# philgzl/brever

Measured on AMD Instinct MI355X. Metric: utterances/sec (4 s @16 kHz) Conv-TasNet train, higher is better.
Workload: dtype bf16

## Files before the change

### brever_amd/csrc/common.cuh

```cuda
#pragma once
#include <hip/hip_runtime.h>
#include <stdint.h>

namespace brv {

typedef __attribute__((ext_vector_type(8))) __bf16 bf16x8;
typedef __attribute__((ext_vector_type(4))) __bf16 bf16x4;
typedef __attribute__((ext_vector_type(4))) short s16x4;
typedef __attribute__((ext_vector_type(16))) float f32x16;
typedef __attribute__((ext_vector_type(4))) float f32x4;

typedef uint16_t bf16_t;

constexpr int kWave = 64;
constexpr int kThreads = 256;

__device__ __forceinline__ float bf2f(bf16_t v) {
  return __uint_as_float(((uint32_t)v) << 16);
}
__device__ __forceinline__ bf16_t f2bf(float f) {
  __bf16 h = (__bf16)f;
  return __builtin_bit_cast(bf16_t, h);
}
typedef __bf16 bf16x2_t __attribute__((ext_vector_type(2)));
// ... 37 lines not shown
__device__ __forceinline__ uint4 buf_load16(__amdgpu_buffer_rsrc_t r, unsigned int off) {
  const u32x4 v = __builtin_amdgcn_raw_buffer_load_b128(r, (int)off, 0, 0);
  return make_uint4(v.x, v.y, v.z, v.w);
}
__device__ __forceinline__ void buf_store16(__amdgpu_buffer_rsrc_t r, unsigned int off, const uint4& q) {
  u32x4 v; v.x = q.x; v.y = q.y; v.z = q.z; v.w = q.w;
#ifndef BRV_STORE_AUX
#define BRV_STORE_AUX 0
#endif
  __builtin_amdgcn_raw_buffer_store_b128(v, r, (int)off, 0, BRV_STORE_AUX);
}
constexpr unsigned int kOob = 0xfffffff0u;

template <typename T>
__device__ __forceinline__ T wave_sum(T v) {
#pragma unroll
  for (int off = 32; off > 0; off >>= 1) v += __shfl_xor(v, off, 64);
  return v;
}

template <typename T>
__device__ __forceinline__ T block_sum(T v, T* scratch) {
  v = wave_sum(v);
  const int lane = threadIdx.x & 63, wid = threadIdx.x >> 6;
  __syncthreads();
  if (lane == 0) scratch[wid] = v;
  __syncthreads();
  T r = T(0);
  if (threadIdx.x == 0) r = scratch[0] + scratch[1] + scratch[2] + scratch[3];
  return r;
}

#ifndef BRV_NO_ATOMICS
#define BRV_NO_ATOMICS 0
#endif
__device__ __forceinline__ void atomic_add_f64(double* p, double v) {
  if (BRV_NO_ATOMICS & 1) return;
  __hip_atomic_fetch_add(p, v, __ATOMIC_RELAXED, __HIP_MEMORY_SCOPE_AGENT);
}
__device__ __forceinline__ void atomic_add_f32(float* p, float v) {
  if (BRV_NO_ATOMICS & 2) return;
  __hip_atomic_fetch_add(p, v, __ATOMIC_RELAXED, __HIP_MEMORY_SCOPE_AGENT);
}

constexpr int kStatStride = 32;
__host__ __device__ __forceinline__ constexpr long long stat_sum(long long b) { return b*kStatStride; }
__host__ __device__ __forceinline__ constexpr long long stat_sq(long long b) { return b*kStatStride + kStatStride/2; }
struct NormStat { float mean, rstd; };
__device__ __forceinline__ float rstd_f32(double v) {
  const float x = (float)v;
  const float r = __builtin_amdgcn_rsqf(x);
  return r*__builtin_fmaf(-0.5f*x*r, r, 1.5f);
}
__device__ __forceinline__ NormStat norm_stat(const double* stats, int b,
                                              double inv_n, float eps) {
  const double s = stats[stat_sum(b)], ss = stats[stat_sq(b)];
  const double mean = s*inv_n;
  double var = ss*inv_n - mean*mean;
  if (var < 0.0) var = 0.0;
  NormStat r;
  r.mean = (float)mean;
  r.rstd = rstd_f32(var + (double)eps);
  return r;
}

__device__ __forceinline__ void load8_masked(const float* p, int c0, int C, float (&v)[8]) {
  if (p != nullptr && c0 + 8 <= C) {
#pragma unroll
    for (int j = 0; j < 8; ++j) v[j] = p[c0 + j];
  } else if (p != nullptr) {
#pragma unroll
    for (int j = 0; j < 8; ++j) {
      const int c = c0 + j;
      const float x = p[c < C ? c : (C > 0 ? C - 1 : 0)];
      v[j] = c < C ? x : 0.f;
    }
  } else {
#pragma unroll
    for (int j = 0; j < 8; ++j) v[j] = 0.f;
  }
}

__host__ __device__ inline int round_up(int x, int m) { return (x + m - 1)/m*m; }
__host__ __device__ inline int ceil_div(int x, int m) { return (x + m - 1)/m; }

}

#define GRID_STRIDE(i, n) \
  for (long long i = (long long)blockIdx.x*256 + threadIdx.x; i < (n); i += (long long)gridDim.x*256)
```

### brever_amd/csrc/convtasnet.hip

```cpp
#include <hip/hip_runtime.h>
#include <stdio.h>
#include <stdlib.h>
#include <string.h>
#include <algorithm>
#include <string>
#include <vector>

#include "../../include/brever_hip.h"
#include "status.h"
#include "ctn_layout.h"
#include "gemm_rows.cuh"
#include "gemm_wgrad.cuh"
#include "gemm_ws.cuh"
#include "dwpw2_fused.cuh"
#include "gemm_wgrad_full.cuh"
#include "gemm_wgrad_full128.cuh"

constexpr int kWgSplit = 4;
#include "prep.cuh"
#include "tcn_kernels.cuh"
#include "bwd_fused.cuh"
#include "pw1_bwd.cuh"
#include "cln_kernels.cuh"

using namespace brv;

namespace {

inline long long align_up(long long x, long long a) { return (x + a - 1)/a*a; }

const brv_launch_opts kDefaultOpts = {sizeof(brv_launch_opts), 0u, 8, 0, nullptr};
thread_local const brv_launch_opts* t_opts = &kDefaultOpts;
struct OptsScope {
  const brv_launch_opts* prev;
  explicit OptsScope(const brv_launch_opts* o) : prev(t_opts) {
    t_opts = (o && o->size >= sizeof(brv_launch_opts)) ? o : &kDefaultOpts;
  }
  ~OptsScope() { t_opts = prev; }
  int check() const {
    const uint32_t unknown = t_opts->flags & ~BRV_OPT_KNOWN;
    if (!unknown) return 0;
    char bits[16]; snprintf(bits, sizeof(bits), "0x%x", unknown);
    return fail(-1, std::string("unknown option bits ") + bits + " in brv_launch_opts.flags");
  }
};
inline bool opt(uint32_t flag) { return (t_opts->flags & flag) != 0; }
inline bool fwd_fuse_requested() { return !opt(BRV_OPT_NO_FWD_FUSE) && !opt(BRV_OPT_NO_WS); }
inline bool bwd_fuse_requested() { return !opt(BRV_OPT_NO_BWD_FUSE); }
inline bool pw1_rc_requested() { return !opt(BRV_OPT_NO_PW1_RC) && !opt(BRV_OPT_NO_DZ1_FUSE); }
inline bool pw1_rc_wgrad() { return opt(BRV_OPT_PW1_RC_WGRAD) || opt(BRV_OPT_PW1_RC_TILES); }

struct ProfEntry { const char* label; hipEvent_t a, b; double flops, bytes; };
struct Prof { std::vector<ProfEntry> entries; bool by_dil; };
struct ProfScope {
  hipStream_t st; Prof* prof;
  ProfScope(const char* label, double flops, double bytes, hipStream_t s)
      : st(s), prof(static_cast<Prof*>(t_opts->prof)) {
    if (!prof) return;
    ProfEntry e; e.label = label; e.flops = flops; e.bytes = bytes;
    (void)hipEventCreate(&e.a); (void)hipEventCreate(&e.b);
    (void)hipEventRecord(e.a, st);
    prof->entries.push_back(e);
  }
  ~ProfScope() { if (prof) (void)hipEventRecord(prof->entries.back().b, st); }
};
inline bool prof_by_dil() { return t_opts->prof && static_cast<Prof*>(t_opts->prof)->by_dil; }

struct BlockOff : CtnBlockOff {
  long long p_c1_f, p_c1_b, p_rs_f, p_rs_b;
  long long p_c1_fp, p_rs_fp, p_rs_bp;
  long long p_rs_g, p_rs_gp, p_lazy;
};

struct Layout : CtnLayout<BlockOff> {
  int Np, Kfp, Bnp, Hp, Scp;
  long long p_enc, p_dec_f, p_dec_b, p_bott_f, p_bott_b, p_out_f, p_out_b, p_stamp, n_prepared;

  bool fusable() const {
    return !causal && P == 3 && H == 512 && Bn == 128 && Sc == 128 && nb <= 24 ;
  }
  bool fused_fwd() const { return fusable() && fwd_fuse_requested(); }
  bool pw1_rc() const { return !causal && Hp == RC_H && Bnp == RC_N && pw1_rc_requested(); }

  static int limits(const brv_ctn_config* c) {
    return c->kernel_size < 1 || c->kernel_size > 5 ? fail(-2, "kernel_size must be in [1, 5] in the HIP path") : 0;
  }
  int init(const brv_ctn_config* c) {
    if (int r = CtnLayout::init(c, limits)) return r;
    Np = round_up(N, 64); Kfp = round_up(K, 64); Bnp = round_up(Bn, 64);
    Hp = round_up(H, 64); Scp = round_up(Sc, 64);
    long long q = 0;
    auto ptake = [&](long long n) { long long r = q; q += align_up(n, 128); return r; };
    p_enc = ptake((long long)Np*Kfp);
    p_dec_f = ptake((long long)Kfp*Np);
    p_dec_b = ptake((long long)Np*Kfp);
    p_bott_f = ptake((long long)Bnp*Np);
    p_bott_b = ptake((long long)Np*Bnp);
    for (int i = 0; i < nb; ++i) {
      const int rs = (i < nb - 1 ? Bnp : 0) + Scp;
      blk[i].p_c1_f = ptake((long long)Hp*Bnp);
      blk[i].p_c1_b = ptake((long long)Bnp*Hp);
      blk[i].p_rs_f = ptake((long long)rs*Hp);
      blk[i].p_rs_b = ptake((long long)Hp*rs);
      blk[i].p_c1_fp = ptake((long long)Hp*Bnp);
      blk[i].p_rs_fp = ptake((long long)rs*Hp);
      blk[i].p_rs_bp = ptake((long long)Hp*rs);
      blk[i].p_rs_g = ptake((long long)(Bnp + Scp)*Hp);
      blk[i].p_rs_gp = ptake((long long)(Bnp + Scp)*Hp);
      blk[i].p_lazy = ptake(4LL*(Bnp + Scp));
    }
    p_out_f = ptake((long long)S*Np*Scp);
    p_out_b = ptake((long long)Scp*S*Np);
    p_stamp = ptake(128);
    n_prepared = q;
    return 0;
  }
};

struct Workspace {
  long long w, x, z1, z2, skip, m, y, stats, sums, dpre, dw1, gskip, gout, eA, eB,
      e0, dwt, vg, gcopy, total;
  long long gcopy_stride, eB_stride;
  long long wgpart;
  long long h1, h2, wn, ctab, ctab_stride, cfs, cbt, ident, fake_stats, scratch_stats;
  long long vg_stride, vg_bytes;
  long long x_stride, z_stride;
  long long u, u_stride;
  long long stamp;
  long long stats_bytes;
  void init(const Layout& l, long long B, long long T) {
    long long o = 0;
    auto take = [&](long long bytes) { long long r = o; o += align_up(bytes, 256); return r; };
    const long long BT = B*T;
    w = take(BT*l.Np*2);
    x_stride = align_up(BT*l.Bnp*2, 256);
    x = take(x_stride*l.nb);
    z_stride = align_up(BT*l.Hp*2, 256);
    z1 = take(z_stride*l.nb);
    z2 = take(z_stride*l.nb);
    skip = take(BT*l.Scp*4);
    m = take(BT*l.S*l.Np*2);
    y = take(BT*l.S*l.Np*2);
    stats_bytes = (long long)(1 + 2*l.nb)*B*kStatStride*8;
    stats = take(stats_bytes);
    sums = take(stats_bytes);
    dpre = take(BT*l.S*l.Np*2);
    dw1 = take(BT*l.S*l.Np*2);
    gout = take(BT*(l.Bnp + l.Scp)*2);
    gskip = gout + (long long)l.Bnp*2;
    eA = take(BT*l.Hp*2);
    eB_stride = align_up(BT*l.Hp*2, 256);
    eB = take(eB_stride*l.nb);
    gcopy_stride = align_up(BT*l.Bnp*2, 256);
    gcopy = take(gcopy_stride*l.nb);
    e0 = take(BT*l.Np*2);
    dwt = take(BT*l.Np*2);
    vg_stride = align_up(2LL*l.N + (long long)l.nb*l.H*(5 + l.P) + 1 + 2*l.nb + 2LL*l.Hp, 64);
    vg_bytes = vg_stride*kReplicas*4;
    vg = take(vg_bytes);
    wgpart = take((long long)2*kWgSplit*l.nb*W2_G*l.H*4);
    u_stride = align_up(BT*(l.Bnp + l.Scp)*2, 256);
    u = l.fusable() ? take(u_stride*l.nb) : 0;
// ... 978 lines not shown
    g.e.src = v.z2(i); g.e.ld_src = l.Hp; g.e.src_slope = params + b.prelu2;
    g.e.src_stats = v.stat(2 + 2*i); g.e.inv_n = 1.0/((double)T*l.H); g.e.eps = 1e-8f;
    g.e.gamma = params + b.n2_g;
    g.e.dgamma = v.vslot(i) + 2*l.H; g.e.dbeta = v.vslot(i) + 3*l.H;
    g.e.rep_stride = v.ws.vg_stride; g.e.n_rep = kReplicas;
    g.e.sums_out = v.sum(2 + 2*i);
    if (int r = launch_gemm_rows<A_BF16, E_GLN_BWD>(g, B, st, "pw2_dgrad", 2.0*BT*(rs0 + l.Scp + 2*l.Hp))) return r;
  }
  const bool fuse_dz2 = blk_fused || (!opt(BRV_OPT_NO_DZ_FUSE) && l.Hp % HL_CG == 0 &&
                        (((l.P - 1)*dil)/2) % dil == 0 && hl_window_rows(dil, l.P) <= HL_MAXROWS);
  DzParams dz; memset(&dz, 0, sizeof(dz));
  if (!fuse_dz2) {
    dz.e = v.eA(); dz.z = v.z2(i); dz.B = B; dz.T = (int)T; dz.Cp = l.Hp; dz.C = l.H;
    dz.slope = params + b.prelu2; dz.stats = v.stat(2 + 2*i); dz.sums = v.sum(2 + 2*i);
    dz.inv_n = 1.0/((double)T*l.H); dz.eps = 1e-8f; dz.dslope = v.vslope() + 2 + 2*i; dz.rep_stride = v.ws.vg_stride;
    if (int r = launch_dz(dz, st)) return r;
  }
  DwParams d; memset(&d, 0, sizeof(d));
  bf16_t* eB = v.eB(i);
  d.z1 = v.z1(i); d.dz2 = v.eA(); d.e1 = eB; d.B = B; d.T = (int)T; d.Cp = l.Hp; d.C = l.H;
  d.slope1 = params + b.prelu1; d.stats1 = v.stat(1 + 2*i);
  d.gamma1 = params + b.n1_g; d.beta1 = params + b.n1_b;
  d.inv_n = 1.0/((double)T*l.H); d.eps = 1e-8f;
  d.taps = params + b.dconv_w; d.dil = dil; d.left = ((l.P - 1)*dil)/2;
  d.dgamma1 = v.vslot(i); d.dbeta1 = v.vslot(i) + l.H;
  d.dtaps = v.vslot(i) + 4*l.H; d.dbias = v.vslot(i) + 4*l.H + (long long)l.H*l.P;
  d.rep_stride = v.ws.vg_stride; d.sums1 = v.sum(1 + 2*i);
  if (fuse_dz2) {
    d.z2in = v.z2(i); d.stats2 = v.stat(2 + 2*i); d.sums2 = v.sum(2 + 2*i);
    d.slope2 = params + b.prelu2; d.dslope2 = v.vslope() + 2 + 2*i;
  }
  if (blk_fused) {
    BwdFusedParams bf; memset(&bf, 0, sizeof(bf));
    bf.d = d; bf.d.dz2 = nullptr;
    bf.g = has_res ? v.gout() : v.gskip(); bf.ldg = ldg; bf.Kg = rs0 + l.Scp;
    bf.Wp = v.prep + b.p_rs_bp; bf.gamma2 = params + b.n2_g;
    bf.dgamma2 = v.vslot(i) + 2*l.H; bf.dbeta2 = v.vslot(i) + 3*l.H;
    if (int r = DwBwdFused<3>::run(bf, st)) return r;
  } else
  if (int r = dispatch_p<DwBwd>(l.P, d, st)) return r;
  return 0;
}

int backward_block_pw1_rc(const Views& v, const float* params, int i, const EpiSpec& e, bool bwd_fused,
                          hipStream_t st) {
  const Layout& l = v.l; const int B = v.B; const long long T = v.T; const double BT = v.BT();
  const BlockOff& b = l.blk[i];
  const bool has_res = i < l.nb - 1;
  bf16_t* eB = v.eB(i);
  Pw1DgradRcParams rp; memset(&rp, 0, sizeof(rp));
  rp.e1 = eB; rp.lde = l.Hp; rp.bse = T*l.Hp;
  rp.x = v.x(i); rp.ldx = l.Bnp; rp.bsx = T*l.Bnp;
  rp.Wfp = v.prep + b.p_c1_fp; rp.bias = params + b.conv_b; rp.Wb = v.prep + b.p_c1_b;
  rp.stats = v.stat(1 + 2*i); rp.sums = v.sum(1 + 2*i); rp.slope = params + b.prelu1;
  rp.inv_n = 1.0/((double)T*l.H); rp.eps = 1e-8f; rp.C = l.H;
  rp.T = (int)T; rp.n_ttiles = ceil_div((int)T, RC_BM); rp.batch = B;
  rp.e = e;
  rp.e.dslope = v.vslope() + 1 + 2*i; rp.e.rep_stride = v.ws.vg_stride; rp.e.n_rep = kReplicas;
  if (opt(BRV_OPT_PW1_RC_TILES)) {
    ProfScope prof("pw1_dgrad", 2.0*BT*(double)l.Hp*l.Bnp*2,
                   2.0*BT*(l.Hp + l.Bnp*(has_res ? 3 : 2)), st);
    hipLaunchKernelGGL(pw1_dgrad_rc_kernel, dim3(rp.n_ttiles*B), dim3(256), 0, st, rp);
  } else {
    Pw1DgradWsParams wp; wp.r = rp;
    wp.dz_out = pw1_rc_wgrad() ? nullptr : eB;
    wp.dbg = nullptr;
#ifdef WSD_STAMP
    wp.dbg = debug_buffer();
#endif
    const double companions = (i > 0 ? l.Bnp : 0) + (bwd_fused && i > 0 ? (double)l.Bnp + 2.0*l.Scp : 0.0);
    ProfScope prof("pw1_dgrad", 2.0*BT*(double)l.Hp*l.Bnp*2,
                   2.0*BT*(l.Hp*(wp.dz_out ? 2 : 1) + l.Bnp*(has_res ? 3 : 2) + companions), st);
    int grid = num_cus();
    const int total = ceil_div((int)T, WSD_TF)*B;
    if (grid > total) grid = total;
    if (l.H == RC_H) hipLaunchKernelGGL(pw1_dgrad_ws_kernel<true>, dim3(grid), dim3(512), 0, st, wp);
    else hipLaunchKernelGGL(pw1_dgrad_ws_kernel<false>, dim3(grid), dim3(512), 0, st, wp);
  }
  BRV_HIP_OK(hipGetLastError());
  return 0;
}

int backward_block_pw1(const Views& v, const float* params, int i, bool bwd_fused, hipStream_t st) {
  const Layout& l = v.l; const int B = v.B; const long long T = v.T; const double BT = v.BT();
  const BlockOff& b = l.blk[i];
  const bool has_res = i < l.nb - 1;
  const int ldg = v.ldg(); bf16_t* eB = v.eB(i); GemmRowsParams g; DzParams dz;
  const bool fuse_dz1 = !opt(BRV_OPT_NO_DZ1_FUSE) && (l.Bnp == 128 || l.Bnp == 64);
  if (!fuse_dz1) {
    memset(&dz, 0, sizeof(dz));
    dz.e = eB; dz.z = v.z1(i); dz.B = B; dz.T = (int)T; dz.Cp = l.Hp; dz.C = l.H;
    dz.slope = params + b.prelu1; dz.stats = v.stat(1 + 2*i); dz.sums = v.sum(1 + 2*i);
    dz.inv_n = 1.0/((double)T*l.H); dz.eps = 1e-8f; dz.dslope = v.vslope() + 1 + 2*i; dz.rep_stride = v.ws.vg_stride;
    if (int r = launch_dz(dz, st)) return r;
  }
  memset(&g, 0, sizeof(g));
  g.a = rows_bf16(eB, l.Hp, T);
  g.W = v.prep + b.p_c1_b; g.T = (int)T; g.Np = l.Bnp; g.Kp = l.Hp;
  g.e.out = v.gout(); g.e.ldo = ldg; g.e.add_in = has_res ? v.gout() : nullptr; g.e.ld_add = ldg;
  g.e.out2 = i > 0 ? v.gcopy(i - 1) : nullptr; g.e.ld_srcf = l.Bnp;
  if (bwd_fused && i > 0) {
    g.e.gu_u = v.u(i - 1); g.e.ld_gu = ldg; g.e.gu_gskip = v.gskip(); g.e.ld_gs = ldg;
    g.e.gu_v1 = reinterpret_cast<const float*>(v.prep + l.blk[i - 1].p_lazy) + ldg;
    g.e.gu_out = v.sum(2 + 2*(i - 1));
  }
  if (fuse_dz1 && l.pw1_rc()) return backward_block_pw1_rc(v, params, i, g.e, bwd_fused, st);
// ... 256 lines not shown
  add(l.dec_w, l.p_dec_b, l.N, l.K, l.Np, l.Kfp, l.Kfp, 0);
  add(l.bott_w, l.p_bott_f, l.Bn, l.N, l.Bnp, l.Np, l.Np, 0);
  add(l.bott_w, l.p_bott_b, l.Bn, l.N, l.Np, l.Bnp, l.Bnp, 1);
  for (int i = 0; i < l.nb; ++i) {
    const BlockOff& b = l.blk[i];
    const bool has_res = i < l.nb - 1;
    const int rs0 = has_res ? l.Bnp : 0, rs = rs0 + l.Scp;
    add(b.conv_w, b.p_c1_f, l.H, l.Bn, l.Hp, l.Bnp, l.Bnp, 0);
    add(b.conv_w, b.p_c1_b, l.H, l.Bn, l.Bnp, l.Hp, l.Hp, 1);
    if (has_res) add(b.res_w, b.p_rs_b, l.Bn, l.H, l.Hp, l.Bnp, rs, 1);
    add(b.skip_w, b.p_rs_b + rs0, l.Sc, l.H, l.Hp, l.Scp, rs, 1);
    if (fused) {
      add(has_res ? b.res_w : 0, b.p_rs_g, has_res ? l.Bn : 0, l.H, l.Bnp, l.Hp, l.Hp, 0);
      jobs.back().scale_off = b.n2_g;
      add(b.skip_w, b.p_rs_g + (long long)l.Bnp*l.Hp, l.Sc, l.H, l.Scp, l.Hp, l.Hp, 0);
      jobs.back().scale_off = b.n2_g;
    } else {
      if (has_res) add(b.res_w, b.p_rs_f, l.Bn, l.H, l.Bnp, l.Hp, l.Hp, 0);
      add(b.skip_w, b.p_rs_f + (long long)rs0*l.Hp, l.Sc, l.H, l.Scp, l.Hp, l.Hp, 0);
    }
  }
  for (int s = 0; s < l.S; ++s) {
    add(l.out_w + (long long)s*l.N*l.Sc, l.p_out_f + (long long)s*l.Np*l.Scp,
        l.N, l.Sc, l.Np, l.Scp, l.Scp, 0);
    add(l.out_w + (long long)s*l.N*l.Sc, l.p_out_b + (long long)s*l.Np,
        l.N, l.Sc, l.Scp, l.Np, l.S*l.Np, 1);
  }
  for (size_t i = 0; i < jobs.size(); i += kPrepBatch) {
    PrepBatch pb;
    pb.n = (int)std::min<size_t>(kPrepBatch, jobs.size() - i);
    for (int k = 0; k < pb.n; ++k) {
      const PrepJob& j = jobs[i + k];
      if (j.src_off > 0x7fffffffLL || j.dst_off > 0x7fffffffLL || j.scale_off > 0x7fffffffLL ||
          (j.R | j.C | j.rows | j.cols | j.dst_ld) > 0xffff)
        return fail(-1, "prepare: layout too large for the compact job form");
      PrepJobC& c = pb.jobs[k];
      c.src_off = (int)j.src_off; c.dst_off = (int)j.dst_off; c.scale_off = (int)j.scale_off;
      c.R = (unsigned short)j.R; c.C = (unsigned short)j.C; c.rows = (unsigned short)j.rows;
      c.cols = (unsigned short)j.cols; c.dst_ld = (unsigned short)j.dst_ld; c.tr = (unsigned short)j.tr;
    }
    hipLaunchKernelGGL(prep_weights_kernel, dim3(8, pb.n), dim3(256), 0, st, params,
                       (bf16_t*)prepared, pb);
    BRV_HIP_OK(hipGetLastError());
  }
  std::vector<PackJob> packs;
  auto pack = [&](long long src, long long dst, int N, int K, int nsl) {
    if (N % nsl || K % 16) return;
    PackJob j; j.src_off = src; j.dst_off = dst; j.N = N; j.K = K; j.nsl = nsl; packs.push_back(j);
  };
  for (int i = 0; i < l.nb; ++i) {
    const BlockOff& b = l.blk[i];
    const int rs = (i < l.nb - 1 ? l.Bnp : 0) + l.Scp;
    pack(b.p_c1_f, b.p_c1_fp, l.Hp, l.Bnp, 64);
    pack(b.p_rs_b, b.p_rs_bp, l.Hp, rs, 32);
    if (fused) pack(b.p_rs_g, b.p_rs_gp, l.Bnp + l.Scp, l.Hp, 32);
    else pack(b.p_rs_f, b.p_rs_fp, rs, l.Hp, 32);
  }
  for (size_t i = 0; i < packs.size(); i += 96) {
    PackBatch pb;
    pb.n = (int)std::min<size_t>(96, packs.size() - i);
    for (int k = 0; k < pb.n; ++k) pb.jobs[k] = packs[i + k];
    hipLaunchKernelGGL(pack_frag_kernel, dim3(16, pb.n), dim3(256), 0, st, (bf16_t*)prepared, pb);
    BRV_HIP_OK(hipGetLastError());
  }
  if (fused) {
    LazyPrepParams lp; memset(&lp, 0, sizeof(lp));
    lp.nb = l.nb; lp.H = l.H; lp.Hp = l.Hp; lp.Bn = l.Bn; lp.Sc = l.Sc; lp.Bnp = l.Bnp; lp.Scp = l.Scp;
    for (int i = 0; i < l.nb; ++i) {
      const BlockOff& b = l.blk[i];
      lp.blk[i].res_w = b.res_w; lp.blk[i].res_b = b.res_b; lp.blk[i].skip_w = b.skip_w;
      lp.blk[i].skip_b = b.skip_b; lp.blk[i].beta = b.n2_b; lp.blk[i].wg = b.p_rs_g; lp.blk[i].out = b.p_lazy;
    }
    lp.stamp = reinterpret_cast<int*>((bf16_t*)prepared + l.p_stamp); lp.stamp_value = mode_stamp(fused);
    hipLaunchKernelGGL(lazy_prep_kernel, dim3((l.Bnp + l.Scp + 3)/4, l.nb), dim3(256), 0, st, params,
                       (bf16_t*)prepared, lp);
    BRV_HIP_OK(hipGetLastError());
  } else {
    hipLaunchKernelGGL(stamp_write_kernel, dim3(1), dim3(1), 0, st,
                       reinterpret_cast<int*>((bf16_t*)prepared + l.p_stamp), mode_stamp(fused));
    BRV_HIP_OK(hipGetLastError());
  }
  return 0;
}

int brv_ctn_forward(const brv_ctn_config* cfg, const float* params, const void* prepared,
                    void* workspace, const float* wave, int64_t wave_stride, float* out, int64_t batch,
                    int64_t length, const brv_launch_opts* opts, brv_stream_t stream) {
  OptsScope scope(opts);
  if (int r = scope.check()) return r;
  if (wave_stride != 0 && wave_stride < length) return fail(-1, "wave_stride shorter than the rows");
  Layout l; if (int r = l.init(cfg)) return r;
  hipStream_t st = (hipStream_t)stream;
  const int B = (int)batch; const long long L = length;
  const long long T = l.frames(L);
  if (B < 1 || T < 1) return fail(-1, "empty batch or input shorter than one frame");
  const Views v(l, workspace, prepared, B, T);
  if (l.causal) return forward_causal(v, params, wave, wave_stride, out, L, st);
  if (int r = forward_encoder(v, params, wave, wave_stride, out, L, st)) return r;

  if (l.fused_fwd()) {
    for (int i = 0; i < l.nb; ++i)
      if (int r = forward_block_fused(v, params, i, st)) return r;
    if (int r = forward_skip_combine(v, st)) return r;
  } else {
    for (int i = 0; i < l.nb; ++i)
      if (int r = forward_block_plain(v, params, i, st)) return r;
// ... 73 lines not shown
```

### brever_amd/csrc/pw1_bwd.cuh

```cuda
#pragma once
#include "gemm_rows.cuh"
#include "gemm_wgrad.cuh"
#include "gfx950.cuh"

namespace brv {

struct Pw1DgradRcParams {
  const bf16_t* e1; int lde; long long bse;
  const bf16_t* x; int ldx; long long bsx;
  const bf16_t* Wfp;
  const float* bias;
  const bf16_t* Wb;
  const double* stats; const double* sums; const float* slope; double inv_n; float eps; int C;
  int T, n_ttiles, batch;
  EpiSpec e;
};

constexpr int RC_BM = 128, RC_BK = 64, RC_LDK = RC_BK + 8, RC_N = 128, RC_H = 512, RC_KX = 128;
constexpr int RC_LDC = RC_N + 4;
constexpr int RC_SMEM_MAIN = 2*RC_BM*RC_LDK*2;
constexpr int RC_SMEM_EPI = RC_BM*RC_LDC*4;
constexpr int RC_SMEM = RC_SMEM_MAIN > RC_SMEM_EPI ? RC_SMEM_MAIN : RC_SMEM_EPI;

__global__ __launch_bounds__(256, 2) void pw1_dgrad_rc_kernel(const Pw1DgradRcParams p) {
  __shared__ __attribute__((aligned(16))) unsigned char smem[RC_SMEM];
  __shared__ __attribute__((aligned(16))) float bias_s[RC_H];
  bf16_t* As = reinterpret_cast<bf16_t*>(smem);
  bf16_t* Ws = As + RC_BM*RC_LDK;
  float* Cs = reinterpret_cast<float*>(smem);
  const int tid = threadIdx.x, lane = tid & 63, wid = tid >> 6;
  const int fr = lane & 31, fh = lane >> 5;
  const int vid = xcd_remap(blockIdx.x, gridDim.x);
  const int b = vid / p.n_ttiles;
  const int t0 = (vid % p.n_ttiles)*RC_BM;
  const int T = p.T;

  for (int c = tid; c < RC_H; c += 256) bias_s[c] = c < p.C ? p.bias[c] : 0.f;

  const NormStat ns = norm_stat(p.stats, b, p.inv_n, p.eps);
  const float slope = *p.slope;
  const float dz_m1 = (float)(p.sums[stat_sum(b)]*p.inv_n);
  const float dz_m2 = (float)(p.sums[stat_sq(b)]*p.inv_n);
  float dz_da = 0.f;

  bf16x8 xf[RC_KX/16];
  {
    const __amdgpu_buffer_rsrc_t rx = make_rsrc(p.x + (long long)b*p.bsx, (long long)T*p.ldx*2);
    const unsigned int off = (unsigned int)(t0 + 32*wid + fr)*(unsigned int)(p.ldx*2) + (unsigned int)(fh*16);
#pragma unroll
    for (int s = 0; s < RC_KX/16; ++s) {
      const uint4 q = buf_load16(rx, off + (unsigned int)(s*32));
      xf[s] = __builtin_bit_cast(bf16x8, q);
    }
  }

  const int sub = lane >> 3, kc = lane & 7;
  const __amdgpu_buffer_rsrc_t re = make_rsrc(p.e1 + (long long)b*p.bse, (long long)T*p.lde*2);
  uint4 eraw[4], wraw[4];
  auto load_chunk = [&](int kt) {
#pragma unroll
    for (int ci = 0; ci < 4; ++ci) {
      const unsigned int t = (unsigned int)(t0 + 32*wid + sub + 8*ci);
      eraw[ci] = buf_load16(re, t*(unsigned int)(p.lde*2) + (unsigned int)((kt*RC_BK + kc*8)*2));
    }
#pragma unroll
// ... 126 lines not shown
      unpack8(*reinterpret_cast<const uint4*>(e.gu_u + rowi*e.ld_gu + ncol), ur);
      unpack8(*reinterpret_cast<const uint4*>(e.gu_u + rowi*e.ld_gu + RC_N + ncol), us);
      float d1 = 0.f, d2 = 0.f;
#pragma unroll
      for (int j = 0; j < 8; ++j) {
        d1 = __builtin_fmaf(gr[j], guv[j], d1);
        d1 = __builtin_fmaf(gs[j], guv[8 + j], d1);
        d2 = __builtin_fmaf(gr[j], ur[j], d2);
        d2 = __builtin_fmaf(gs[j], us[j], d2);
      }
      st_sum += d1; st_sq += d2;
    }
  }
  if (e.gu_out) {
    __syncthreads();
    double* dscr = reinterpret_cast<double*>(smem);
    const double s0 = block_sum(st_sum, dscr);
    const double s1 = block_sum(st_sq, dscr + 8);
    if (tid == 0) { atomic_add_f64(e.gu_out + stat_sum(b), s0); atomic_add_f64(e.gu_out + stat_sq(b), s1); }
  }
  {
    __syncthreads();
    float* fscr = reinterpret_cast<float*>(smem);
    const float s0 = block_sum(dz_da, fscr);
    if (tid == 0 && e.dslope) {
      const long long ro = e.n_rep > 1 ? (long long)(blockIdx.x % e.n_rep)*e.rep_stride : 0;
      atomic_add_f32(e.dslope + ro, s0);
    }
  }
}

#ifndef WSD_ABL
#define WSD_ABL 0
#endif
struct Pw1DgradWsParams {
  Pw1DgradRcParams r;
  bf16_t* dz_out;
  long long* dbg;
};
#ifdef WSD_STAMP
#define WSD_MARK(role, idx) do { const long long t_ = stamp_cycles(); \
    if (lane == 0 && pp.dbg && (idx) < 32) pp.dbg[(long long)blockIdx.x*64 + (role)*32 + (idx)] = t_; } while (0)
#else
#define WSD_MARK(role, idx) do { } while (0)
#endif

constexpr int WSD_TF = 32;
constexpr int WSD_LDX = RC_KX + 8;
constexpr int WSD_LDE = 128 + 8;
constexpr int WSD_LDD = RC_H + 8;
constexpr int WSD_LDC = 32 + 4;
constexpr int WSD_XB = WSD_TF*WSD_LDX*2, WSD_EB = WSD_TF*WSD_LDE*2, WSD_DB = WSD_TF*WSD_LDD*2;
constexpr int WSD_CB = WSD_TF*WSD_LDC*4;
constexpr int WSD_SMEM = 2*WSD_XB + 4*WSD_EB + 2*WSD_DB + 4*WSD_CB + RC_H*4 + 2*RC_N*4;
static_assert(WSD_SMEM <= 160*1024, "LDS budget");

template <bool FULLC>
__global__ __launch_bounds__(512) void pw1_dgrad_ws_kernel(const Pw1DgradWsParams pp) {
  const Pw1DgradRcParams& p = pp.r;
  __shared__ __attribute__((aligned(16))) unsigned char smem[WSD_SMEM];
  bf16_t* Xs = reinterpret_cast<bf16_t*>(smem);
  bf16_t* Es = reinterpret_cast<bf16_t*>(smem + 2*WSD_XB);
  bf16_t* Ds = reinterpret_cast<bf16_t*>(smem + 2*WSD_XB + 4*WSD_EB);
  float* Cs_all = reinterpret_cast<float*>(smem + 2*WSD_XB + 4*WSD_EB + 2*WSD_DB);
  float* bias_s = reinterpret_cast<float*>(smem + 2*WSD_XB + 4*WSD_EB + 2*WSD_DB + 4*WSD_CB);
  float* guv_s = bias_s + RC_H;
  const int tid = threadIdx.x, lane = tid & 63;
  const int wid = __builtin_amdgcn_readfirstlane(tid >> 6);
  const int fr = lane & 31, fh = lane >> 5;
  const int T = p.T;
  const EpiSpec& e = p.e;

  for (int c = tid; c < RC_H; c += 512) bias_s[c] = c < p.C ? p.bias[c] : 0.f;
  if (tid < 2*RC_N) guv_s[tid] = e.gu_out ? e.gu_v1[tid] : 0.f;

  const int tpi = ceil_div(T, WSD_TF);
  const int total = tpi*p.batch;
  const int per = ceil_div(total, (int)gridDim.x);
  const int t_begin = blockIdx.x*per;
  const int t_end = min(total, t_begin + per);
  const int t_items = tpi*WSD_TF;
  if (t_begin >= t_end) return;

  auto advance = [&](int& b, int& t) { t += WSD_TF; if (t >= t_items) { t = 0; ++b; } };
  const int n_tiles = t_end - t_begin;
  const int b0 = t_begin / tpi, tf0 = (t_begin % tpi)*WSD_TF;

  if (wid < 4) {
    if (wid == 0) WSD_MARK(0, 0);
    bf16x8 wf[4][8];
    {
      const bf16_t* src = p.Wfp + (long long)wid*128*RC_KX + (long long)lane*8;
#pragma unroll
      for (int f = 0; f < 4; ++f)
#pragma unroll
        for (int s = 0; s < 8; ++s) wf[f][s] = *reinterpret_cast<const bf16x8*>(src + (f*8 + s)*512);
    }
    const float slope = *p.slope;
    const float pc1 = 0.5f*(1.f + slope), pc2 = 0.5f*(1.f - slope);
    float da2 = 0.f;
    int cur_b = -1;
    float rstd = 1.f, dz_m1 = 0.f, dz_m2 = 0.f, XA = 0.f, XB = 0.f, XC = 0.f;
    const int ec = lane & 15, er = lane >> 4;
    bf16_t* es = Es + wid*WSD_TF*WSD_LDE;
    uint4 eraw[8];
    auto load_e = [&](int b, int t0, bool valid) {
      const __amdgpu_buffer_rsrc_t re = make_rsrc(p.e1 + (long long)b*p.bse, (valid && !(WSD_ABL & 4)) ? (long long)T*p.lde*2 : 0);
#pragma unroll
      for (int ci = 0; ci < 8; ++ci)
        eraw[ci] = buf_load16(re, (unsigned int)(t0 + er + 4*ci)*(unsigned int)(p.lde*2)
                                  + (unsigned int)((128*wid + ec*8)*2));
    };
    int b_ld = b0, t_ld = tf0;
    load_e(b_ld, t_ld, true);
    if (wid == 0) WSD_MARK(0, 1);
#pragma unroll 1
    for (int i = 0; i <= n_tiles; ++i) {
      const int buf = i & 1;
      const int b = b_ld, t0 = t_ld;
      if (wid == 0) WSD_MARK(0, 2 + 3*i);
#pragma unroll
      for (int ci = 0; ci < 8; ++ci)
        *reinterpret_cast<uint4*>(es + (er + 4*ci)*WSD_LDE + ec*8) = eraw[ci];
      if (wid == 0) { wait_vm<0>(); WSD_MARK(0, 3 + 3*i); }
      __syncthreads();
      if (wid == 0) WSD_MARK(0, 4 + 3*i);
      if (i == n_tiles) break;
      advance(b_ld, t_ld);
      load_e(b_ld, t_ld, i + 1 < n_tiles);
      if (b != cur_b) {
        const NormStat ns = norm_stat(p.stats, b, p.inv_n, p.eps);
        rstd = ns.rstd;
        XA = pc1*ns.rstd; XB = pc2*ns.rstd; XC = -ns.mean*ns.rstd;
        dz_m1 = (float)(p.sums[stat_sum(b)]*p.inv_n);
        dz_m2 = (float)(p.sums[stat_sq(b)]*p.inv_n);
        cur_b = b;
      }
      const bf16_t* xs = Xs + buf*WSD_TF*WSD_LDX;
      bf16_t* ds = Ds + buf*WSD_TF*WSD_LDD;
      const float R = (t0 + fr < T) ? rstd : 0.f;
      const float K0 = -dz_m1*R, M2 = -dz_m2*R;
#pragma unroll
      for (int f = 0; f < 4; ++f) {
        f32x16 az;
#pragma unroll
        for (int g = 0; g < 4; ++g) {
          const float4 bv = *reinterpret_cast<const float4*>(bias_s + 128*wid + 32*f + 8*g + 4*fh);
          az[4*g] = bv.x; az[4*g + 1] = bv.y; az[4*g + 2] = bv.z; az[4*g + 3] = bv.w;
        }
#pragma unroll
        for (int s = 0; s < 8; ++s) {
          const bf16x8 xb = *reinterpret_cast<const bf16x8*>(xs + fr*WSD_LDX + 16*s + 8*fh);
          if (!(WSD_ABL & 8)) az = __builtin_amdgcn_mfma_f32_32x32x16_bf16(wf[f][s], xb, az, 0, 0, 0);
          else az[s] += __builtin_bit_cast(f32x4, xb)[0] + __builtin_bit_cast(f32x4, wf[f][s])[0];
        }
#pragma unroll
        for (int g = 0; g < 4; ++g) {
          const int kch = 128*wid + 32*f + 8*g + 4*fh;
          const uint2 eq = *reinterpret_cast<const uint2*>(es + fr*WSD_LDE + 32*f + 8*g + 4*fh);
          const float ev[4] = {__uint_as_float(eq.x << 16), __uint_as_float(eq.x & 0xffff0000u),
                               __uint_as_float(eq.y << 16), __uint_as_float(eq.y & 0xffff0000u)};
          const uint32_t zq0 = pack2(az[4*g], az[4*g + 1]), zq1 = pack2(az[4*g + 2], az[4*g + 3]);
          const float zv[4] = {__uint_as_float(zq0 << 16), __uint_as_float(zq0 & 0xffff0000u),
                               __uint_as_float(zq1 << 16), __uint_as_float(zq1 & 0xffff0000u)};
          float o[4];
#pragma unroll
          for (int j = 0; j < 4; ++j) {
            const float z = zv[j];
            if (WSD_ABL & 1) { o[j] = z + ev[j]; continue; }
            const float xh = __builtin_fmaf(XB, __builtin_fabsf(z), __builtin_fmaf(XA, z, XC));
            float dh = __builtin_fmaf(xh, M2, __builtin_fmaf(ev[j], R, K0));
            if (!FULLC) dh = kch + j < p.C ? dh : 0.f;
            o[j] = z > 0.f ? dh : slope*dh;
            da2 = __builtin_fmaf(dh, z - __builtin_fabsf(z), da2);
          }
          uint2 v;
          v.x = pack2(o[0], o[1]); v.y = pack2(o[2], o[3]);
          *reinterpret_cast<uint2*>(ds + fr*WSD_LDD + kch) = v;
        }
      }
    }
    const float dz_da = 0.5f*da2;
    const float s0 = wave_sum(dz_da);
    if (lane == 0 && e.dslope) {
      const long long ro = e.n_rep > 1 ? (long long)((blockIdx.x*4 + wid) % e.n_rep)*e.rep_stride : 0;
      atomic_add_f32(e.dslope + ro, s0);
    }
  } else {
    const int cw = wid - 4;
    bf16x8 wb[32];
    {
      const bf16_t* srb = p.Wb + (long long)(32*cw + fr)*RC_H + 8*fh;
#pragma unroll
      for (int s = 0; s < 32; ++s) wb[s] = *reinterpret_cast<const bf16x8*>(srb + 16*s);
    }
    float* Cw = Cs_all + cw*WSD_TF*WSD_LDC;
    const int orow = lane >> 2, ocol = 32*cw + 8*(lane & 3);
    double gu_s = 0.0, gu_q = 0.0;
    int cur_b = -1;
    auto flush_gu = [&]() {
      if (cur_b < 0 || !e.gu_out) return;
      const double s0 = wave_sum(gu_s), s1 = wave_sum(gu_q);
      if (lane == 0) { atomic_add_f64(e.gu_out + stat_sum(cur_b), s0); atomic_add_f64(e.gu_out + stat_sq(cur_b), s1); }
      gu_s = 0.0; gu_q = 0.0;
    };
    const int ctid = tid - 256;
    uint4 xraw[2];
    auto load_x = [&](int b, int t0, bool valid) {
      const __amdgpu_buffer_rsrc_t rx = make_rsrc(p.x + (long long)b*p.bsx, valid ? (long long)T*p.ldx*2 : 0);
#pragma unroll
      for (int k = 0; k < 2; ++k) {
        const int id = ctid + 256*k;
        xraw[k] = buf_load16(rx, (unsigned int)(t0 + (id >> 4))*(unsigned int)(p.ldx*2) + (unsigned int)((id & 15)*16));
      }
    };
    int b_ld = b0, t_ld = tf0;
    int b_pv = b0, t_pv = tf0;
    load_x(b_ld, t_ld, true);
    if (wid == 4) { WSD_MARK(1, 0); WSD_MARK(1, 1); }
#pragma unroll 1
    for (int i = 0; i <= n_tiles; ++i) {
      const int buf = i & 1;
      if (wid == 4) WSD_MARK(1, 2 + 3*i);
#pragma unroll
      for (int k = 0; k < 2; ++k) {
        const int id = ctid + 256*k;
        *reinterpret_cast<uint4*>(Xs + buf*WSD_TF*WSD_LDX + (id >> 4)*WSD_LDX + (id & 15)*8) = xraw[k];
      }
      const int b = b_pv, t0 = t_pv;
      uint4 c_add[2], c_gs[2], c_ur[2], c_us[2];
#pragma unroll
      for (int k = 0; k < 2; ++k) {
        const int t = t0 + orow + 16*k;
        const long long rowi = (long long)b*T + t;
        c_add[k] = c_gs[k] = c_ur[k] = c_us[k] = make_uint4(0, 0, 0, 0);
        if (i > 0 && t < T && !(WSD_ABL & 2)) {
          if (e.add_in) c_add[k] = *reinterpret_cast<const uint4*>(e.add_in + rowi*e.ld_add + ocol);
          if (e.gu_out) {
            c_gs[k] = *reinterpret_cast<const uint4*>(e.gu_gskip + rowi*e.ld_gs + ocol);
            c_ur[k] = *reinterpret_cast<const uint4*>(e.gu_u + rowi*e.ld_gu + ocol);
            c_us[k] = *reinterpret_cast<const uint4*>(e.gu_u + rowi*e.ld_gu + RC_N + ocol);
          }
        }
      }
      if (wid == 4) WSD_MARK(1, 3 + 3*i);
      __syncthreads();
      if (wid == 4) WSD_MARK(1, 4 + 3*i);
      if (i < n_tiles) {
        advance(b_ld, t_ld);
        load_x(b_ld, t_ld, i + 1 < n_tiles);
      }
      if (i == 0) continue;
      advance(b_pv, t_pv);
      if (b != cur_b) { flush_gu(); cur_b = b; }
      const bf16_t* ds = Ds + (buf ^ 1)*WSD_TF*WSD_LDD;
      if (pp.dz_out != nullptr && !(WSD_ABL & 32)) {
        const __amdgpu_buffer_rsrc_t rd = make_rsrc(pp.dz_out + (long long)b*p.bse, (long long)T*p.lde*2);
#pragma unroll
        for (int ci = 0; ci < 8; ++ci) {
          const int row = 4*ci + cw;
          buf_store16(rd, (unsigned int)(t0 + row)*(unsigned int)(p.lde*2) + (unsigned int)(lane*16),
                      *reinterpret_cast<const uint4*>(ds + row*WSD_LDD + lane*8));
        }
      }
      f32x16 ag;
#pragma unroll
      for (int q = 0; q < 16; ++q) ag[q] = 0.f;
#pragma unroll
      for (int s = 0; s < 32; ++s) {
        const bf16x8 db = *reinterpret_cast<const bf16x8*>(ds + fr*WSD_LDD + 16*s + 8*fh);
        if (!(WSD_ABL & 16)) ag = __builtin_amdgcn_mfma_f32_32x32x16_bf16(wb[s], db, ag, 0, 0, 0);
        else ag[s & 15] += __builtin_bit_cast(f32x4, db)[0] + __builtin_bit_cast(f32x4, wb[s])[0];
      }
#pragma unroll
      for (int g = 0; g < 4; ++g)
        *reinterpret_cast<float4*>(Cw + fr*WSD_LDC + 8*g + 4*fh) =
            make_float4(ag[4*g], ag[4*g + 1], ag[4*g + 2], ag[4*g + 3]);
      __builtin_amdgcn_fence(__ATOMIC_RELEASE, "wavefront");
      __builtin_amdgcn_wave_barrier();
      __builtin_amdgcn_fence(__ATOMIC_ACQUIRE, "wavefront");
#pragma unroll
      for (int k = 0; k < 2; ++k) {
        const int row = orow + 16*k, t = t0 + row;
        if (t >= T) continue;
        const long long rowi = (long long)b*T + t;
        float v[8];
        {
          const float4 lo = *reinterpret_cast<const float4*>(Cw + row*WSD_LDC + 8*(lane & 3));
          const float4 hi = *reinterpret_cast<const float4*>(Cw + row*WSD_LDC + 8*(lane & 3) + 4);
          v[0] = lo.x; v[1] = lo.y; v[2] = lo.z; v[3] = lo.w;
          v[4] = hi.x; v[5] = hi.y; v[6] = hi.z; v[7] = hi.w;
        }
        if (e.add_in) {
          float r[8];
          unpack8(c_add[k], r);
#pragma unroll
          for (int j = 0; j < 8; ++j) v[j] += r[j];
        }
        const uint4 qa = pack8(v);
        if (!(WSD_ABL & 32)) {
          *reinterpret_cast<uint4*>(reinterpret_cast<bf16_t*>(e.out) + rowi*e.ldo + ocol) = qa;
          if (e.out2) *reinterpret_cast<uint4*>(e.out2 + rowi*e.ld_srcf + ocol) = qa;
        } else if (qa.x == 0x12345678u) Cw[0] = 1.f;
        if (e.gu_out && !(WSD_ABL & 2)) {
          float gr[8], gs[8], ur[8], us[8];
// ... 208 lines not shown
```

Before: 2478.

## Prefetch norm stats via consumer waves and pack backward weights for coalesced loads

Consumer waves now prefetch per-batch norm statistics one tile ahead and publish the computed rstd/mean/dz means into a small LDS slot. Producer waves read those values instead of doing serialized global double loads whenever the batch changes. The backward pw1 weights are pre-packed into a lane-contiguous layout so each wave loads its register-resident weight fragment with coalesced strided reads. Bias and gate vector staging is folded into the first tile's barrier, and the loop prologue is peeled. This removes stalls at kernel start and at batch boundaries, but adds LDS traffic and extra prep memory, and the timing of the stats handoff across double buffers is delicate.

```diff
diff --git a/brever_amd/csrc/common.cuh b/brever_amd/csrc/common.cuh
--- a/brever_amd/csrc/common.cuh
+++ b/brever_amd/csrc/common.cuh
@@ -113,9 +113,7 @@
   const float r = __builtin_amdgcn_rsqf(x);
   return r*__builtin_fmaf(-0.5f*x*r, r, 1.5f);
 }
-__device__ __forceinline__ NormStat norm_stat(const double* stats, int b,
-                                              double inv_n, float eps) {
-  const double s = stats[stat_sum(b)], ss = stats[stat_sq(b)];
+__device__ __forceinline__ NormStat norm_stat_of(double s, double ss, double inv_n, float eps) {
   const double mean = s*inv_n;
   double var = ss*inv_n - mean*mean;
   if (var < 0.0) var = 0.0;
@@ -123,6 +121,10 @@
   r.mean = (float)mean;
   r.rstd = rstd_f32(var + (double)eps);
   return r;
+}
+__device__ __forceinline__ NormStat norm_stat(const double* stats, int b,
+                                              double inv_n, float eps) {
+  return norm_stat_of(stats[stat_sum(b)], stats[stat_sq(b)], inv_n, eps);
 }
 
 __device__ __forceinline__ void load8_masked(const float* p, int c0, int C, float (&v)[8]) {
diff --git a/brever_amd/csrc/convtasnet.hip b/brever_amd/csrc/convtasnet.hip
--- a/brever_amd/csrc/convtasnet.hip
+++ b/brever_amd/csrc/convtasnet.hip
@@ -69,6 +69,7 @@
 struct BlockOff : CtnBlockOff {
   long long p_c1_f, p_c1_b, p_rs_f, p_rs_b;
   long long p_c1_fp, p_rs_fp, p_rs_bp;
+  long long p_c1_bp;
   long long p_rs_g, p_rs_gp, p_lazy;
 };
 
@@ -81,6 +82,7 @@
   }
   bool fused_fwd() const { return fusable() && fwd_fuse_requested(); }
   bool pw1_rc() const { return !causal && Hp == RC_H && Bnp == RC_N && pw1_rc_requested(); }
+  bool c1_b_packed() const { return Hp == RC_H && Bnp == RC_N; }
 
   static int limits(const brv_ctn_config* c) {
     return c->kernel_size < 1 || c->kernel_size > 5 ? fail(-2, "kernel_size must be in [1, 5] in the HIP path") : 0;
@@ -108,6 +110,7 @@
       blk[i].p_rs_g = ptake((long long)(Bnp + Scp)*Hp);
       blk[i].p_rs_gp = ptake((long long)(Bnp + Scp)*Hp);
       blk[i].p_lazy = ptake(4LL*(Bnp + Scp));
+      blk[i].p_c1_bp = c1_b_packed() ? ptake((long long)Bnp*Hp) : -1;
     }
     p_out_f = ptake((long long)S*Np*Scp);
     p_out_b = ptake((long long)Scp*S*Np);
@@ -1192,6 +1195,7 @@
   rp.e1 = eB; rp.lde = l.Hp; rp.bse = T*l.Hp;
   rp.x = v.x(i); rp.ldx = l.Bnp; rp.bsx = T*l.Bnp;
   rp.Wfp = v.prep + b.p_c1_fp; rp.bias = params + b.conv_b; rp.Wb = v.prep + b.p_c1_b;
+  rp.Wbp = b.p_c1_bp >= 0 ? v.prep + b.p_c1_bp : nullptr;
   rp.stats = v.stat(1 + 2*i); rp.sums = v.sum(1 + 2*i); rp.slope = params + b.prelu1;
   rp.inv_n = 1.0/((double)T*l.H); rp.eps = 1e-8f; rp.C = l.H;
   rp.T = (int)T; rp.n_ttiles = ceil_div((int)T, RC_BM); rp.batch = B;
@@ -1554,6 +1558,7 @@
     const BlockOff& b = l.blk[i];
     const int rs = (i < l.nb - 1 ? l.Bnp : 0) + l.Scp;
     pack(b.p_c1_f, b.p_c1_fp, l.Hp, l.Bnp, 64);
+    if (b.p_c1_bp >= 0) pack(b.p_c1_b, b.p_c1_bp, l.Bnp, l.Hp, 32);
     pack(b.p_rs_b, b.p_rs_bp, l.Hp, rs, 32);
     if (fused) pack(b.p_rs_g, b.p_rs_gp, l.Bnp + l.Scp, l.Hp, 32);
     else pack(b.p_rs_f, b.p_rs_fp, rs, l.Hp, 32);
diff --git a/brever_amd/csrc/pw1_bwd.cuh b/brever_amd/csrc/pw1_bwd.cuh
--- a/brever_amd/csrc/pw1_bwd.cuh
+++ b/brever_amd/csrc/pw1_bwd.cuh
@@ -11,6 +11,7 @@
   const bf16_t* Wfp;
   const float* bias;
   const bf16_t* Wb;
+  const bf16_t* Wbp;
   const double* stats; const double* sums; const float* slope; double inv_n; float eps; int C;
   int T, n_ttiles, batch;
   EpiSpec e;
@@ -243,7 +244,7 @@
 constexpr int WSD_LDC = 32 + 4;
 constexpr int WSD_XB = WSD_TF*WSD_LDX*2, WSD_EB = WSD_TF*WSD_LDE*2, WSD_DB = WSD_TF*WSD_LDD*2;
 constexpr int WSD_CB = WSD_TF*WSD_LDC*4;
-constexpr int WSD_SMEM = 2*WSD_XB + 4*WSD_EB + 2*WSD_DB + 4*WSD_CB + RC_H*4 + 2*RC_N*4;
+constexpr int WSD_SMEM = 2*WSD_XB + 4*WSD_EB + 2*WSD_DB + 4*WSD_CB + RC_H*4 + 2*RC_N*4 + 2*4*4;
 static_assert(WSD_SMEM <= 160*1024, "LDS budget");
 
 template <bool FULLC>
@@ -256,14 +257,12 @@
   float* Cs_all = reinterpret_cast<float*>(smem + 2*WSD_XB + 4*WSD_EB + 2*WSD_DB);
   float* bias_s = reinterpret_cast<float*>(smem + 2*WSD_XB + 4*WSD_EB + 2*WSD_DB + 4*WSD_CB);
   float* guv_s = bias_s + RC_H;
+  float* nrm_s = guv_s + 2*RC_N;
   const int tid = threadIdx.x, lane = tid & 63;
   const int wid = __builtin_amdgcn_readfirstlane(tid >> 6);
   const int fr = lane & 31, fh = lane >> 5;
   const int T = p.T;
   const EpiSpec& e = p.e;
-
-  for (int c = tid; c < RC_H; c += 512) bias_s[c] = c < p.C ? p.bias[c] : 0.f;
-  if (tid < 2*RC_N) guv_s[tid] = e.gu_out ? e.gu_v1[tid] : 0.f;
 
   const int tpi = ceil_div(T, WSD_TF);
   const int total = tpi*p.batch;
@@ -279,19 +278,6 @@
 
   if (wid < 4) {
     if (wid == 0) WSD_MARK(0, 0);
-    bf16x8 wf[4][8];
-    {
-      const bf16_t* src = p.Wfp + (long long)wid*128*RC_KX + (long long)lane*8;
-#pragma unroll
-      for (int f = 0; f < 4; ++f)
-#pragma unroll
-        for (int s = 0; s < 8; ++s) wf[f][s] = *reinterpret_cast<const bf16x8*>(src + (f*8 + s)*512);
-    }
-    const float slope = *p.slope;
-    const float pc1 = 0.5f*(1.f + slope), pc2 = 0.5f*(1.f - slope);
-    float da2 = 0.f;
-    int cur_b = -1;
-    float rstd = 1.f, dz_m1 = 0.f, dz_m2 = 0.f, XA = 0.f, XB = 0.f, XC = 0.f;
     const int ec = lane & 15, er = lane >> 4;
     bf16_t* es = Es + wid*WSD_TF*WSD_LDE;
     uint4 eraw[8];
@@ -302,8 +288,21 @@
         eraw[ci] = buf_load16(re, (unsigned int)(t0 + er + 4*ci)*(unsigned int)(p.lde*2)
                                   + (unsigned int)((128*wid + ec*8)*2));
     };
+    const float bias_v = p.bias[min(tid, p.C - 1)];
+    const float slope = *p.slope;
+    bf16x8 wf[4][8];
+    {
+      const bf16_t* src = p.Wfp + (long long)wid*128*RC_KX + (long long)lane*8;
+#pragma unroll
+      for (int f = 0; f < 4; ++f)
+#pragma unroll
+        for (int s = 0; s < 8; ++s) wf[f][s] = *reinterpret_cast<const bf16x8*>(src + (f*8 + s)*512);
+    }
     int b_ld = b0, t_ld = tf0;
     load_e(b_ld, t_ld, true);
+    const float pc1 = 0.5f*(1.f + slope), pc2 = 0.5f*(1.f - slope);
+    float da2 = 0.f;
+    float rstd = 1.f, dz_m1 = 0.f, dz_m2 = 0.f, XA = 0.f, XB = 0.f, XC = 0.f;
     if (wid == 0) WSD_MARK(0, 1);
 #pragma unroll 1
     for (int i = 0; i <= n_tiles; ++i) {
@@ -313,19 +312,16 @@
 #pragma unroll
       for (int ci = 0; ci < 8; ++ci)
         *reinterpret_cast<uint4*>(es + (er + 4*ci)*WSD_LDE + ec*8) = eraw[ci];
+      if (i == 0) bias_s[tid] = tid < p.C ? bias_v : 0.f;
       if (wid == 0) { wait_vm<0>(); WSD_MARK(0, 3 + 3*i); }
       __syncthreads();
       if (wid == 0) WSD_MARK(0, 4 + 3*i);
       if (i == n_tiles) break;
       advance(b_ld, t_ld);
       load_e(b_ld, t_ld, i + 1 < n_tiles);
-      if (b != cur_b) {
-        const NormStat ns = norm_stat(p.stats, b, p.inv_n, p.eps);
-        rstd = ns.rstd;
-        XA = pc1*ns.rstd; XB = pc2*ns.rstd; XC = -ns.mean*ns.rstd;
-        dz_m1 = (float)(p.sums[stat_sum(b)]*p.inv_n);
-        dz_m2 = (float)(p.sums[stat_sq(b)]*p.inv_n);
-        cur_b = b;
+      if (i == 0 || t0 == 0) {
+        const float4 n = *reinterpret_cast<const float4*>(nrm_s + 4*buf);
+        rstd = n.x; XA = pc1*n.x; XB = pc2*n.x; XC = n.y; dz_m1 = n.z; dz_m2 = n.w;
       }
       const bf16_t* xs = Xs + buf*WSD_TF*WSD_LDX;
       bf16_t* ds = Ds + buf*WSD_TF*WSD_LDD;
@@ -379,12 +375,6 @@
     }
   } else {
     const int cw = wid - 4;
-    bf16x8 wb[32];
-    {
-      const bf16_t* srb = p.Wb + (long long)(32*cw + fr)*RC_H + 8*fh;
-#pragma unroll
-      for (int s = 0; s < 32; ++s) wb[s] = *reinterpret_cast<const bf16x8*>(srb + 16*s);
-    }
     float* Cw = Cs_all + cw*WSD_TF*WSD_LDC;
     const int orow = lane >> 2, ocol = 32*cw + 8*(lane & 3);
     double gu_s = 0.0, gu_q = 0.0;
@@ -408,16 +398,57 @@
     int b_ld = b0, t_ld = tf0;
     int b_pv = b0, t_pv = tf0;
     load_x(b_ld, t_ld, true);
+    const float bias_v = p.bias[min(tid, p.C - 1)];
+    const float guv_v = e.gu_out ? e.gu_v1[ctid] : 0.f;
+    double sraw[4] = {0.0, 0.0, 0.0, 0.0};
+    auto load_stats = [&](int b) {
+      if (cw != 0) return;
+      sraw[0] = p.stats[stat_sum(b)]; sraw[1] = p.stats[stat_sq(b)];
+      sraw[2] = p.sums[stat_sum(b)]; sraw[3] = p.sums[stat_sq(b)];
+    };
+    auto publish_stats = [&](int i) {
+      if (cw != 0) return;
+      const NormStat ns = norm_stat_of(sraw[0], sraw[1], p.inv_n, p.eps);
+      if (lane == 0)
+        *reinterpret_cast<float4*>(nrm_s + 4*(i & 1)) =
+            make_float4(ns.rstd, -ns.mean*ns.rstd, (float)(sraw[2]*p.inv_n), (float)(sraw[3]*p.inv_n));
+    };
+    load_stats(b0);
+    bf16x8 wb[32];
+    if (p.Wbp != nullptr) {
+      const bf16_t* srb = p.Wbp + (long long)cw*32*RC_H + (long long)lane*8;
+#pragma unroll
+      for (int s = 0; s < 32; ++s) wb[s] = *reinterpret_cast<const bf16x8*>(srb + s*512);
+    } else {
+      const bf16_t* srb = p.Wb + (long long)(32*cw + fr)*RC_H + 8*fh;
+#pragma unroll
+      for (int s = 0; s < 32; ++s) wb[s] = *reinterpret_cast<const bf16x8*>(srb + 16*s);
+    }
     if (wid == 4) { WSD_MARK(1, 0); WSD_MARK(1, 1); }
-#pragma unroll 1
-    for (int i = 0; i <= n_tiles; ++i) {
-      const int buf = i & 1;
+    auto stage_x = [&](int i) {
       if (wid == 4) WSD_MARK(1, 2 + 3*i);
 #pragma unroll
       for (int k = 0; k < 2; ++k) {
         const int id = ctid + 256*k;
-        *reinterpret_cast<uint4*>(Xs + buf*WSD_TF*WSD_LDX + (id >> 4)*WSD_LDX + (id & 15)*8) = xraw[k];
-      }
+        *reinterpret_cast<uint4*>(Xs + (i & 1)*WSD_TF*WSD_LDX + (id >> 4)*WSD_LDX + (id & 15)*8) = xraw[k];
+      }
+    };
+    stage_x(0);
+    bias_s[tid] = tid < p.C ? bias_v : 0.f;
+    guv_s[ctid] = guv_v;
+    publish_stats(0);
+    if (wid == 4) WSD_MARK(1, 3);
+    __syncthreads();
+    if (wid == 4) WSD_MARK(1, 4);
+    advance(b_ld, t_ld);
+    load_x(b_ld, t_ld, 1 < n_tiles);
+    bool opens = 1 < n_tiles && t_ld == 0;
+    if (opens) load_stats(b_ld);
+#pragma unroll 1
+    for (int i = 1; i <= n_tiles; ++i) {
+      const int buf = i & 1;
+      stage_x(i);
+      if (opens) publish_stats(i);
       const int b = b_pv, t0 = t_pv;
       uint4 c_add[2], c_gs[2], c_ur[2], c_us[2];
 #pragma unroll
@@ -425,7 +456,7 @@
         const int t = t0 + orow + 16*k;
         const long long rowi = (long long)b*T + t;
         c_add[k] = c_gs[k] = c_ur[k] = c_us[k] = make_uint4(0, 0, 0, 0);
-        if (i > 0 && t < T && !(WSD_ABL & 2)) {
+        if (t < T && !(WSD_ABL & 2)) {
           if (e.add_in) c_add[k] = *reinterpret_cast<const uint4*>(e.add_in + rowi*e.ld_add + ocol);
           if (e.gu_out) {
             c_gs[k] = *reinterpret_cast<const uint4*>(e.gu_gskip + rowi*e.ld_gs + ocol);
@@ -437,11 +468,13 @@
       if (wid == 4) WSD_MARK(1, 3 + 3*i);
       __syncthreads();
       if (wid == 4) WSD_MARK(1, 4 + 3*i);
+      opens = false;
       if (i < n_tiles) {
         advance(b_ld, t_ld);
         load_x(b_ld, t_ld, i + 1 < n_tiles);
-      }
-      if (i == 0) continue;
+        opens = i + 1 < n_tiles && t_ld == 0;
+        if (opens) load_stats(b_ld);
+      }
       advance(b_pv, t_pv);
       if (b != cur_b) { flush_gu(); cur_b = b; }
       const bf16_t* ds = Ds + (buf ^ 1)*WSD_TF*WSD_LDD;
```

Result: no change. 2506 (median of 2 runs) (+1.1%).
